# alibaba/PhotonLibOS

Measured on AMD Instinct MI355X. Metric: GiB/s CRC32C over device-resident buffers; % of HBM-read roofline, higher is better.
Workload: dtype u8; 1 GPU; C2: 65536 x 64 KiB random buffers, device-resident, per GPU; config=c2, buffers=65536, buffer_bytes=65536, parallelism=shard-per-gpu x1, lanes_per_buffer=auto

## Files before the change

### include/photon_crc/tuning.h

```cpp
#ifndef PHOTON_CRC_TUNING_H
#define PHOTON_CRC_TUNING_H

#include <stdint.h>

#ifdef __cplusplus
extern "C" {
#endif

int photon_crc_set_lanes_per_buffer(int g);

int photon_crc_set_batch_grid(int workgroups);

int photon_crc_set_generic_rows(int rows_per_step);

int photon_crc_set_msg_mode(int mode);

int photon_crc_set_msg_rows(int rows_per_step);

int photon_crc_set_mid_kernel(int on);

int photon_crc_set_long_shape(int lanes, int rounds);

int photon_crc64_set_full_rows(int mode, int rows_per_step);

int photon_crc_set_routed_wait(int spin_us, int sleep_ahead);

int photon_crc_set_small_service(int idle_us);
int photon_crc_set_small_service_life(int life_us);
int photon_crc_set_service_doorbell(int bar);
int photon_crc_small_service_doorbell(int kind);
int photon_crc_small_service_stats(uint64_t* served, uint64_t* starts, uint64_t* missed);
uint64_t photon_crc_small_service_deferred(void);

int photon_crc_lanes_for(uint64_t nbytes);

void photon_crc_test_fail_next(int n);

int photon_crc_test_tables(int which, uint32_t* out, int n);

int photon_crc_test_long_plan(uint64_t addr, uint64_t n, int cus, int lanes, int rounds, int crc64, uint64_t* out,
                              int nout);

int photon_crc_test_fold_parts(int crc64, const void* crc, const uint64_t* len, uint64_t count, uint64_t seed,
                               uint32_t nthreads, uint64_t* result, uint64_t* total);

int photon_crc_util_fold_on_host(int crc64, const void* d_crc, const uint64_t* h_len, const uint64_t* h_obj_start,
                                 uint64_t nobj, uint64_t nparts, uint64_t seed, void* h_out, void* stream);

int photon_crc_util_fill_splitmix(void* d_base, uint64_t stride, uint64_t nbytes, uint64_t count,
                                  uint64_t seed_base, void* stream);

int photon_crc_util_read_stream(const void* d_base, uint64_t nbytes, uint32_t* d_sink, uint64_t sink_words,
                                void* stream);

#ifdef __cplusplus
}
#endif

#endif
```

### photonlibos_amd/_native.py

```python
import ctypes
import os

_HERE = os.path.dirname(os.path.abspath(__file__))
LIB_PATH = os.environ.get("PHOTON_CRC_LIB") or os.path.join(_HERE, "lib", "libphoton_checksum.so")

_lib = None


class NativeLibraryMissing(ImportError):
    pass


class PhotonRange(ctypes.Structure):
    _fields_ = [("min", ctypes.c_int), ("max", ctypes.c_int)]


def lib():
    global _lib
    if _lib is None:
        if not os.path.exists(LIB_PATH):
            raise NativeLibraryMissing(
                f"{LIB_PATH} not found: build it with `python -c 'import __graft_entry__ as g; g.build()'` "
                "(or `make -C photonlibos_amd/csrc`)")
        _lib = ctypes.CDLL(LIB_PATH, mode=ctypes.RTLD_GLOBAL)
        _declare(_lib)
    return _lib


def _declare(L):
    u8p, u32, u64, sz, vp = ctypes.c_char_p, ctypes.c_uint32, ctypes.c_uint64, ctypes.c_size_t, ctypes.c_void_p
    u32p = ctypes.POINTER(ctypes.c_uint32)

    def fn(name, res, *args):
        f = getattr(L, name)
        f.restype = res
        f.argtypes = list(args)

    fn("photon_crc_device_count", ctypes.c_int)
    fn("photon_crc_last_error", ctypes.c_char_p)
    fn("photon_crc_scratch_release", ctypes.c_int64)
    fn("photon_crc_set_lanes_per_buffer", ctypes.c_int, ctypes.c_int)
    fn("photon_crc_set_batch_grid", ctypes.c_int, ctypes.c_int)
    fn("photon_crc32c_batch_strided", ctypes.c_int, vp, u64, u64, u64, u32, vp, vp, vp)
    fn("photon_crc32c_batch_strided_sync", ctypes.c_int, vp, u64, u64, u64, u32, vp, vp, vp)
    fn("photon_crc32c_batch_iov", ctypes.c_int, vp, u64, u32, vp, vp, vp)
    fn("photon_crc32c_host_batch_strided", ctypes.c_int, vp, u64, u64, u64, u32, vp, vp)
    fn("photon_crc32c_host_batch_strided_multi", ctypes.c_int, vp, u64, u64, u64, u32, vp, vp, ctypes.c_int)
    fn("photon_crc32c_batch_strided_shards", ctypes.c_int, vp, ctypes.c_int)
    fn("photon_crc32c_batch_msg", ctypes.c_int, vp, vp, u64, u32, vp, vp, vp, vp)
    fn("photon_crc32c_combine_batch", ctypes.c_int, vp, vp, vp, u64, vp, vp)
    fn("photon_crc64ecma_batch_strided", ctypes.c_int, vp, u64, u64, u64, u64, vp, vp, vp)
    fn("photon_crc64ecma_batch_iov", ctypes.c_int, vp, u64, u64, vp, vp, vp)
    fn("photon_crc64ecma_host_batch_strided", ctypes.c_int, vp, u64, u64, u64, u64, vp, vp)
    fn("photon_crc64ecma_trim_batch", ctypes.c_int, vp, vp, vp, u64, vp, vp, vp)
    fn("photon_crc64ecma_combine_batch", ctypes.c_int, vp, vp, vp, u64, vp, vp)
    fn("photon_crc64ecma_batch_msg_n", ctypes.c_int, vp, vp, u64, u64, u64, vp, vp, vp, vp)
    fn("photon_crc64ecma_extend_device", ctypes.c_int, vp, u64, u64, vp, vp)
    fn("photon_crc_util_fill_splitmix", ctypes.c_int, vp, u64, u64, u64, u64, vp)
    fn("photon_crc_util_read_stream", ctypes.c_int, vp, u64, vp, u64, vp)
    fn("photon_crc_set_generic_rows", ctypes.c_int, ctypes.c_int)
    fn("photon_crc_set_long_shape", ctypes.c_int, ctypes.c_int, ctypes.c_int)
    fn("photon_crc_set_msg_mode", ctypes.c_int, ctypes.c_int)
    fn("photon_crc_set_routed_wait", ctypes.c_int, ctypes.c_int, ctypes.c_int)
    fn("photon_crc_set_small_service", ctypes.c_int, ctypes.c_int)
    fn("photon_crc_set_mid_kernel", ctypes.c_int, ctypes.c_int)
    fn("photon_crc_small_service_stats", ctypes.c_int, vp, vp, vp)
    fn("photon_crc_set_small_service_life", ctypes.c_int, ctypes.c_int)
    fn("photon_crc_set_service_doorbell", ctypes.c_int, ctypes.c_int)
    fn("photon_crc_small_service_doorbell", ctypes.c_int, ctypes.c_int)
    fn("photon_crc_small_service_deferred", u64)
    fn("photon_crc64_set_full_rows", ctypes.c_int, ctypes.c_int, ctypes.c_int)
    fn("photon_crc_host_register", ctypes.c_int, vp, u64)
    fn("photon_crc_stream_create", ctypes.c_int, ctypes.POINTER(vp))
    fn("photon_crc_stream_destroy", ctypes.c_int, vp)
    fn("photon_crc_stream_sync", ctypes.c_int, vp)
    fn("photon_crc_stream_on_complete", ctypes.c_int, vp, vp, vp)
    fn("photon_crc_device_alloc", ctypes.c_int, ctypes.POINTER(vp), u64)
    fn("photon_crc_device_free", ctypes.c_int, vp)
    fn("photon_crc_memcpy_async", ctypes.c_int, vp, vp, u64, vp)
    fn("photon_crc_host_unregister", ctypes.c_int, vp)
    fn("photon_crc32c_file_strided", ctypes.c_int, ctypes.c_int, u64, u64, u64, u64, u32, vp)
    fn("photon_crc_dispatch_fallbacks", u64)
    fn("photon_crc_lanes_for", ctypes.c_int, u64)
    fn("photon_crc_test_fail_next", None, ctypes.c_int)
    fn("photon_crc_test_long_plan", ctypes.c_int, u64, u64, ctypes.c_int, ctypes.c_int, ctypes.c_int, ctypes.c_int,
       vp, ctypes.c_int)
    fn("photon_crc32c_series_device", ctypes.c_int, vp, u32, u32, vp, vp)
    fn("photon_crc32c_combine_series_device", ctypes.c_int, vp, u32, u32, vp, vp)
    fn("photon_crc32c_trim_batch", ctypes.c_int, vp, vp, vp, u64, vp, vp, vp)
    fn("photon_crc32c_extend_device", ctypes.c_int, vp, u64, u32, vp, vp)
    fn("photon_crc32c_extend_spans", ctypes.c_int, vp, ctypes.c_int, u32, vp)
    fn("photon_crc64ecma_extend_spans", ctypes.c_int, vp, ctypes.c_int, u64, vp)
    fn("photon_crc_set_device_dispatch", ctypes.c_int, ctypes.c_int)
    fn("photon_crc32c_batch_msg_n", ctypes.c_int, vp, vp, u64, u64, u32, vp, vp, vp, vp)
    fn("photon_crc32c_copy_batch_strided", ctypes.c_int, vp, u64, vp, u64, u64, u64, u32, vp, vp, vp)
    fn("photon_crc32c_copy_batch_iov", ctypes.c_int, vp, vp, u64, u32, vp, vp, vp)
    fn("photon_crc32c_gather_msg_n", ctypes.c_int, vp, vp, u64, u64, vp, u32, vp, vp, vp, vp)
    fn("photon_crc64ecma_copy_batch_strided", ctypes.c_int, vp, u64, vp, u64, u64, u64, u64, vp, vp, vp)
    fn("photon_crc64ecma_copy_batch_iov", ctypes.c_int, vp, vp, u64, u64, vp, vp, vp)
    fn("photon_crc64ecma_gather_msg_n", ctypes.c_int, vp, vp, u64, u64, vp, u64, vp, vp, vp, vp)
    fn("photon_crc32c_copy_msg_iov_n", ctypes.c_int, vp, vp, u64, vp, vp, u64, u64, vp, u32, vp, vp, vp, vp)
    fn("photon_crc64ecma_copy_msg_iov_n", ctypes.c_int, vp, vp, u64, vp, vp, u64, u64, vp, u64, vp, vp, vp, vp)
    fn("photon_crc32c_copy_msg_iov_seg_n", ctypes.c_int, vp, vp, u64, vp, vp, u64, u64, vp, u32, vp, ctypes.c_int, vp,
       vp, vp, vp)
    fn("photon_crc64ecma_copy_msg_iov_seg_n", ctypes.c_int, vp, vp, u64, vp, vp, u64, u64, vp, u64, vp, ctypes.c_int,
       vp, vp, vp, vp)
    fn("photon_crc32c_copy_extend_device", ctypes.c_int, vp, vp, u64, u32, vp, vp)
    fn("photon_crc64ecma_copy_extend_device", ctypes.c_int, vp, vp, u64, u64, vp, vp)
    fn("photon_crc64ecma_series_device", ctypes.c_int, vp, u32, u32, vp, vp)
    fn("photon_crc64ecma_combine_series_device", ctypes.c_int, vp, u32, u32, vp, vp)
    fn("photon_crc32c_fold_parts_n", ctypes.c_int, vp, vp, vp, u64, u64, u32, vp, vp, vp, vp)
    fn("photon_crc64ecma_fold_parts_n", ctypes.c_int, vp, vp, vp, u64, u64, u64, vp, vp, vp, vp)
    fn("photon_crc_test_fold_parts", ctypes.c_int, ctypes.c_int, vp, vp, u64, u64, u32, vp, vp)
    fn("photon_crc_util_fold_on_host", ctypes.c_int, ctypes.c_int, vp, vp, vp, u64, u64, u64, vp, vp)
    fn("photon_crc_pinned_allocate", ctypes.c_int, vp, PhotonRange, ctypes.POINTER(vp))
    fn("photon_crc_pinned_deallocate", ctypes.c_int, vp, vp)
    fn("photon_crc_pinned_stats", ctypes.c_int, ctypes.POINTER(u64), ctypes.POINTER(u64))
    fn("photon_crc_pinned_release", ctypes.c_int64)
    fn("photon_crc_msg_batch_create", vp, u32, u32, u32)
    fn("photon_crc_msg_batch_destroy", None, vp)
    fn("photon_crc_msg_batch_add", ctypes.c_int64, vp, vp, u32, vp, u64, u32)
    fn("photon_crc_msg_batch_submit", ctypes.c_int, vp, vp, vp, vp)
    fn("photon_crc_msg_batch_wait", ctypes.c_int64, vp)
    fn("photon_crc_msg_batch_result", ctypes.c_int, vp, u64, ctypes.POINTER(u32))
    fn("photon_crc_msg_batch_count", u64, vp)
    fn("photon_crc_msg_batch_reset", ctypes.c_int, vp)

    cpp = {
        "crc32c_sw": ("_Z9crc32c_swPKhmj", u32, u8p, sz, u32),
        "crc32c_hw": ("_Z9crc32c_hwPKhmj", u32, u8p, sz, u32),
        "crc32c_hw_simple": ("_Z16crc32c_hw_simplePKhmj", u32, u8p, sz, u32),
        "crc32c_hw_portable": ("_Z18crc32c_hw_portablePKhmj", u32, u8p, sz, u32),
        "crc32c_series_sw": ("_Z16crc32c_series_swPKhjjPj", None, u8p, u32, u32, u32p),
        "crc32c_series_hw": ("_Z16crc32c_series_hwPKhjjPj", None, u8p, u32, u32, u32p),
        "crc32c_combine_sw": ("_Z17crc32c_combine_swjjj", u32, u32, u32, u32),
        "crc32c_combine_hw": ("_Z17crc32c_combine_hwjjj", u32, u32, u32, u32),
        "crc32c_combine_series_sw": ("_Z24crc32c_combine_series_swPjjj", u32, u32p, u32, u32),
        "crc32c_combine_series_hw": ("_Z24crc32c_combine_series_hwPjjj", u32, u32p, u32, u32),
        "crc32c_trim_sw": ("_Z14crc32c_trim_sw16CRC32C_ComponentS_S_", u32, u64, u64, u64),
        "crc32c_trim_hw": ("_Z14crc32c_trim_hw16CRC32C_ComponentS_S_", u32, u64, u64, u64),
        "crc64ecma_sw": ("_Z12crc64ecma_swPKhmm", u64, u8p, sz, u64),
        "crc64ecma_hw": ("_Z12crc64ecma_hwPKhmm", u64, u8p, sz, u64),
        "crc64ecma_series_sw": ("_Z19crc64ecma_series_swPKhjjPm", None, u8p, u32, u32, ctypes.POINTER(u64)),
        "crc64ecma_series_hw": ("_Z19crc64ecma_series_hwPKhjjPm", None, u8p, u32, u32, ctypes.POINTER(u64)),
        "crc64ecma_combine_sw": ("_Z20crc64ecma_combine_swmmj", u64, u64, u64, u32),
        "crc64ecma_combine_hw": ("_Z20crc64ecma_combine_hwmmj", u64, u64, u64, u32),
        "crc64ecma_combine_series_sw": ("_Z27crc64ecma_combine_series_swPmjj", u64, ctypes.POINTER(u64), u32, u32),
        "crc64ecma_combine_series_hw": ("_Z27crc64ecma_combine_series_hwPmjj", u64, ctypes.POINTER(u64), u32, u32),
        "crc64ecma_trim_sw": ("_Z17crc64ecma_trim_sw19CRC64ECMA_ComponentS_S_", u64, u64, u64, u64, u64, u64, u64),
        "crc64ecma_trim_hw": ("_Z17crc64ecma_trim_hw19CRC64ECMA_ComponentS_S_", u64, u64, u64, u64, u64, u64, u64),
    }
    L.cpp = {}
    for py, (mangled, res, *args) in cpp.items():
        f = getattr(L, mangled)
# ... 9 lines not shown
```

### photonlibos_amd/checksum.py

```python
import ctypes

from ._native import lib

__all__ = [
    "CrcError",
    "crc32c", "crc32c_extend", "crc32c_sw", "crc32c_hw", "crc32c_hw_simple", "crc32c_hw_portable",
    "crc32c_series", "crc32c_series_sw", "crc32c_series_hw",
    "crc32c_combine", "crc32c_combine_sw", "crc32c_combine_hw",
    "crc32c_combine_series", "crc32c_combine_series_sw", "crc32c_combine_series_hw",
    "crc32c_trim", "crc32c_trim_sw", "crc32c_trim_hw", "is_crc32c_hw_available",
    "device_count", "set_lanes_per_buffer", "host_batch_strided", "host_batch_strided_multi", "batch_strided_shards",
    "Shard", "batch_strided", "batch_strided_sync", "batch_iov", "batch_msg",
    "copy_batch_strided", "copy_batch_iov", "gather_msg_n",
    "crc64ecma", "crc64ecma_extend", "crc64ecma_sw", "crc64ecma_hw", "crc64ecma_combine", "crc64ecma_series",
    "crc64ecma_combine_series", "crc64ecma_trim",
    "copy_batch64_strided", "copy_batch64_iov", "gather64_msg_n",
    "copy_msg_iov_n", "copy_msg64_iov_n",
    "copy_msg_iov_seg_n", "copy_msg64_iov_seg_n", "SEG_OF_SRC", "SEG_OF_DST",
    "copy_extend_device", "copy_extend64_device",
    "series64_device", "combine_series64_device", "fold_parts_device", "fold_parts64_device",
    "crc64ecma_series_at", "crc64ecma_combine_series_at",
    "batch64_strided", "batch64_iov", "combine64_batch", "trim64_batch", "batch64_msg_n", "host_batch64_strided", "extend64_device", "extend_spans", "extend64_spans", "Span", "combine_batch", "fill_splitmix", "read_stream", "IOVEC_DTYPE",
]

# ... 490 lines not shown


_SERIES64_PTR_FN = _SERIES_PTR_FN
_CSER64_PTR_FN = ctypes.CFUNCTYPE(ctypes.c_uint64, ctypes.c_void_p, ctypes.c_uint32, ctypes.c_uint32)


def crc64ecma_series_at(addr, part_size, n_parts, out_addr):
    _auto("crc64ecma_series_auto", _SERIES64_PTR_FN)(addr, part_size, n_parts, out_addr)


def crc64ecma_combine_series_at(addr, part_size, n_parts):
    return _auto("crc64ecma_combine_series_auto", _CSER64_PTR_FN)(addr, part_size, n_parts)


def host_register(addr, nbytes):
    _check(lib().photon_crc_host_register(addr, nbytes))


def host_unregister(addr):
    _check(lib().photon_crc_host_unregister(addr))


def file_strided(fd, offset, stride, nbytes, count, seed=0):
    out = (ctypes.c_uint32 * max(count, 1))()
    _check(lib().photon_crc32c_file_strided(fd, offset, stride, nbytes, count, seed & 0xFFFFFFFF, out))
    return list(out)[:count]


def set_generic_rows(u):
    _check(lib().photon_crc_set_generic_rows(u))


def set_msg_mode(mode):
    _check(lib().photon_crc_set_msg_mode(mode))


def set_long_shape(lanes=0, rounds=0):
    _check(lib().photon_crc_set_long_shape(lanes, rounds))


def set_routed_wait(spin_us=40, sleep_ahead=True):
    _check(lib().photon_crc_set_routed_wait(spin_us, 1 if sleep_ahead else 0))


def set_mid_kernel(on=True):
    _check(lib().photon_crc_set_mid_kernel(1 if on else 0))


def set_small_service(idle_us):
    _check(lib().photon_crc_set_small_service(int(idle_us)))


def set_small_service_life(life_us):
    _check(lib().photon_crc_set_small_service_life(int(life_us)))


def set_service_doorbell(bar):
    _check(lib().photon_crc_set_service_doorbell(1 if bar else 0))


def small_service_doorbell(kind=0):
    r = lib().photon_crc_small_service_doorbell(int(kind))
    if r == -2:
        return None
    _check(r if r < 0 else 0)
    return "bar" if r == 1 else "pinned"


def small_service_deferred():
    return int(lib().photon_crc_small_service_deferred())


def small_service_stats():
    import ctypes
    v = [ctypes.c_uint64(0) for _ in range(3)]
    _check(lib().photon_crc_small_service_stats(*[ctypes.byref(x) for x in v]))
    return tuple(x.value for x in v)


def set_full_rows64(mode, rows_per_step=2):
    _check(lib().photon_crc64_set_full_rows(mode, rows_per_step))


def set_msg_rows(u):
    _check(lib().photon_crc_set_msg_rows(u))


def read_stream(base, nbytes, sink, sink_words, stream=None):
    _check(lib().photon_crc_util_read_stream(_ptr(base), nbytes, _ptr(sink), sink_words, _stream(stream)))


def fill_splitmix(base, stride, nbytes, count, seed_base, stream=None):
    _check(lib().photon_crc_util_fill_splitmix(_ptr(base), stride, nbytes, count, seed_base, _stream(stream)))


def scratch_release():
    return int(lib().photon_crc_scratch_release())
```

### photonlibos_amd/csrc/crc32c_device.hip

```cpp
#include <hip/hip_runtime.h>

#include <errno.h>
#include <fcntl.h>
#include <stdint.h>
#include <stdio.h>
#include <string.h>

#include <sys/prctl.h>
#include <unistd.h>

#include <atomic>
#include <chrono>
#include <memory>
#include <map>
#include <tuple>
#include <mutex>
#include <string>
#include <thread>
#include <type_traits>
#include <vector>

#include <photon/common/checksum/crc32c.h>
#include <photon/common/checksum/crc64ecma.h>

#include "../../include/photon_crc/crc32c_gpu.h"
#include "../../include/photon_crc/tuning.h"
#include "crc32c_kernels.h"
#include "crc64_kernels.h"
#include "long_plan.h"
#include "multi_device.h"
#include "gf2.h"
#include "internal.h"

namespace pcrc {
int host_engine_table(int which, uint32_t* out, int n);

namespace {

thread_local std::string g_err;

std::atomic<int> g_lanes_override{0};
std::atomic<int> g_grid_cap{0};
std::atomic<int> g_generic_u{-1};
std::atomic<int> g_msg_u{2};
std::atomic<int> g_msg_mode{0};
std::atomic<uint32_t> g_full64{2u << 4 | 3u};
std::atomic<uint32_t> g_routed_wait{40u | 1u << 16};
constexpr int kSvcIdleDefault = 200;
int svc_idle_from_env() {
    const char* e = getenv("PHOTON_CRC_SMALL_SERVICE");
    if (!e || !*e) return kSvcIdleDefault;
    const long v = strtol(e, nullptr, 10);
    return v < 0 ? 0 : v > 1000000 ? 1000000 : (int)v;
}
std::atomic<int> g_svc_idle_us{svc_idle_from_env()};
std::atomic<int> g_svc_life_us{2000};
int svc_bell_from_env() {
    const char* e = getenv("PHOTON_CRC_SVC_DOORBELL");
    return e && (!strcmp(e, "host") || !strcmp(e, "pinned") || !strcmp(e, "0")) ? 0 : 1;
}
std::atomic<int> g_svc_bell{svc_bell_from_env()};
std::atomic<uint64_t> g_svc_served{0}, g_svc_starts{0}, g_svc_missed{0}, g_svc_deferred{0};
std::atomic<int> g_svc_made{0};
void service_end_all();
void svc_yield();
void heavy_mark(hipStream_t st);

struct HeavyLaunch {
    hipStream_t st;
    explicit HeavyLaunch(hipStream_t s) : st(s) { svc_yield(); }
    ~HeavyLaunch() { heavy_mark(st); }
};
int service_doorbell_of(int dev, int kind);

int fail(int code, const std::string& what) {
    g_err = what;
    return code;
}

int hip_fail(hipError_t e, const char* what, const char* rest = "") {
    return fail(-EIO, std::string(what) + rest + ": " + hipGetErrorString(e));
}

struct HipRT {
    int get(int* dev) {
        const hipError_t e = hipGetDevice(dev);
        return e == hipSuccess ? 0 : hip_fail(e, "hipGetDevice");
    }
    int set(int dev) {
        const hipError_t e = hipSetDevice(dev);
        return e == hipSuccess ? 0 : hip_fail(e, "hipSetDevice");
    }
};

struct DeviceInfo {
    bool probed = false;
    bool ok = false;
    int cus = 0;
};

std::mutex g_mu;
std::vector<DeviceInfo> g_dev;
thread_local int g_fail_next = 0;

void table_images_init();

int current_device(int* cus) {
    if (g_fail_next > 0) {
        --g_fail_next;
        return fail(-EIO, "injected failure (photon_crc_test_fail_next)");
    }
    int dev = 0;
    hipError_t e = hipGetDevice(&dev);
    if (e != hipSuccess) return hip_fail(e, "hipGetDevice");
    std::lock_guard<std::mutex> lk(g_mu);
    if ((int)g_dev.size() <= dev) g_dev.resize(dev + 1);
    DeviceInfo& di = g_dev[dev];
    if (!di.probed) {
        hipDeviceProp_t prop;
        e = hipGetDeviceProperties(&prop, dev);
        if (e != hipSuccess) return hip_fail(e, "hipGetDeviceProperties");
        di.ok = strncmp(prop.gcnArchName, "gfx950", 6) == 0;
        di.cus = prop.multiProcessorCount;
        di.probed = true;
        if (!di.ok) g_err = std::string("device is ") + prop.gcnArchName + ", need gfx950";
        if (di.ok) table_images_init();
    }
    if (!di.ok) return fail(-ENODEV, "photon_crc: no gfx950 device (got other arch)");
    *cus = di.cus;
// ... 108 lines not shown
    c.kshift = xpow(8ull * 16ull * (uint64_t)b * (uint64_t)g);
    mul_basis(c.kshift, c.sbasis);
    for (int k = 0; k < 6; ++k) mul_basis(xpow((128ull * (uint64_t)b) << k), c.basis[k]);
    for (int d = 0; d < 8; ++d) mul_basis(xpow(32ull + 128ull * (uint64_t)d), c.fbasis[d]);
    return c;
}

const LaneConsts& lane_consts(int g, int b = 1) {
    static LaneConsts tab[7][3];
    static std::once_flag once;
    std::call_once(once, [] {
        for (int lg = 2; lg <= 6; ++lg)
            for (int lb = 0; lb <= 2; ++lb) tab[lg][lb] = make_lane_consts(1 << lg, 1 << lb);
    });
    const int lg = g == 64 ? 6 : g == 32 ? 5 : g == 16 ? 4 : g == 8 ? 3 : 2;
    const int lb = b == 4 ? 2 : b == 2 ? 1 : 0;
    return tab[lg][lb];
}

LaneConsts64 make_lane_consts64(int g) {
    LaneConsts64 c;
    c.kshift = xpow64(8ull * 16ull * (uint64_t)g);
    for (int i = 0; i < 64; ++i) c.sbasis[i] = mulmod64(1ull << i, c.kshift);
    return c;
}

const LaneConsts64& lane_consts64(int g) {
    static LaneConsts64 tab[7];
    static std::once_flag once;
    std::call_once(once, [] {
        for (int lg = 2; lg <= 6; ++lg) tab[lg] = make_lane_consts64(1 << lg);
    });
    return tab[g == 64 ? 6 : g == 32 ? 5 : g == 16 ? 4 : g == 8 ? 3 : 2];
}

template <typename W>
typename W::Pow squarings(typename W::T v) {
    typename W::Pow t;
    for (int i = 0; i < 64; ++i) {
        t.x8pow2[i] = v;
        v = W::mul(v, v);
    }
    return t;
}

template <typename W, bool INV>
const typename W::Pow& x8_table() {
    static typename W::Pow t;
    static std::once_flag once;
    std::call_once(once, [] { t = squarings<W>(INV ? W::xpow_inv(8) : W::xpow(8)); });
    return t;
}

template <typename W>
const typename W::Pow& pow_table() {
    return x8_table<W, false>();
}

template <typename W>
const typename W::Pow& rshift_table() {
    return x8_table<W, true>();
}

template <typename W>
typename W::Pow part_pow_table(uint64_t part) {
    return squarings<W>(W::xpow(8ull * part));
}

int choose_lanes(uint64_t typical_len) {
    if (const int g = g_lanes_override.load(std::memory_order_relaxed)) return g;
    if (typical_len >= (512u << 10)) return 64;
    if (typical_len >= (32u << 10)) return 32;
    if (typical_len >= 2048) return 8;
    return 4;
}

int batch_lanes(uint64_t typical_len) {
    if (const int g = g_lanes_override.load(std::memory_order_relaxed)) return g;
    if (typical_len >= 4096 && typical_len < 8192) return 16;
    return choose_lanes(typical_len);
}

constexpr int default_rows(int g) { return g == 16 ? 2 : 4; }

int batch_rows(int g) {
    const int u = g_generic_u.load(std::memory_order_relaxed);
    return u >= 0 ? u : default_rows(g);
}

std::vector<uint32_t> small_image_host();
std::vector<uint64_t> small64_image_host();

struct Crc32c : Gf32 {
    static constexpr const char* kKernel = "crc32c";
    static constexpr const char* kExtend = "crc32c_extend";
    static constexpr const char* kSeries = "crc32c_series";
    static constexpr const char* kCombineSeries = "crc32c_combine_series";
    static constexpr const char* kCombineSeriesLaunch = "combine_series kernel launch";
    static constexpr bool kCrc64 = false;
    static constexpr int kService = 0;
    typedef LaneConsts Lanes;
    typedef PowTable Pow;
    typedef BatchArgs Batch;
    typedef CopyBatchArgs CopyBatch;
    typedef CopyIovArgs CopyIov;
    typedef SmallArgs Small;
    typedef LongArgs Long;
    typedef CopyLongArgs CopyLong;
    static T xpow(uint64_t n) { return pcrc::xpow(n); }
    static T xpow_inv(uint64_t n) { return pcrc::xpow_inv(n); }
    static const Lanes& lanes(int g) { return lane_consts(g); }
    static constexpr bool kShiftInit = PCRC_SHIFT_INIT;
    static T shift_init(T seed0, uint64_t nbytes) { return mul(seed0, xpow(8ull * nbytes)); }
    static int copy_lanes(uint64_t typical_len) { return batch_lanes(typical_len); }
    static constexpr uint32_t kSeriesMinPart = 8;
    static constexpr uint32_t kSeedBytes = 4;
    static void put_seed(Small* a, T seed) { a->seed = seed; }
    static T seed_word(const Small& a) { return a.seed; }
    static constexpr uint32_t kImageBytes = kSmImage;
    static constexpr const char* kImageName = "small-buffer table image";
    static std::vector<T> image_host() { return small_image_host(); }
    static constexpr uint32_t kMidBlocks = pcrc::kMidBlocks, kMidRows = pcrc::kMidRows;
    template <uint32_t V, int R>
    static auto small_kernel() { return &crc32c_small_kernel<V, R>; }
    template <int G>
    static auto long_kernel() { return &crc32c_long_kernel<G, 4>; }
    template <int G>
    static auto copy_long_kernel() { return &crc32c_copy_long_kernel<G, 4>; }
    static void long_args(Long* a, const LongPlan& lp, const LongPowers& pw, const void* data, T seed, T* out) {
        pcrc::long_args(a, lp, pw, data, seed, out);
    }
    static constexpr auto* kCombineKernel = &crc32c_combine_kernel;
    static constexpr auto* kTrimKernel = &crc32c_trim_kernel;
    static constexpr auto* kFoldPartsKernel = &crc32c_fold_parts_kernel;
    static constexpr auto* kCombineSeriesKernel = &crc32c_combine_series_kernel;
    static bool combine_series_of_empty(const T* d_crc, uint32_t part_size, uint32_t n_parts, T* d_result,
                                        hipStream_t st) {
        if (part_size) return false;
        hipLaunchKernelGGL(crc32c_first_nonzero_kernel, dim3(1), dim3(1024), 0, st, d_crc, (uint64_t)n_parts,
                           d_result);
        return true;
    }
    static constexpr uint32_t kWords = 1;
    static T routed_result(const uint32_t* x, bool ) { return x[0]; }
    static void routed_diag(char* buf, size_t n, const volatile uint64_t* w, uint32_t tag) {
        snprintf(buf, n, "; word %016llx, tag %08x", (unsigned long long)w[0], tag);
    }
    static inline T (*host_crc)(const uint8_t*, size_t, T) = nullptr;
    static inline void (*host_series)(const uint8_t*, uint32_t, uint32_t, T*) = nullptr;
    static inline T (*host_cseries)(T*, uint32_t, uint32_t) = nullptr;
};

struct Crc64 : Gf64 {
    static constexpr const char* kKernel = "crc64";
    static constexpr const char* kExtend = "crc64ecma_extend";
    static constexpr const char* kSeries = "crc64ecma_series";
    static constexpr const char* kCombineSeries = "crc64ecma_combine_series";
    static constexpr const char* kCombineSeriesLaunch = "crc64_combine_series_kernel launch";
    static constexpr bool kCrc64 = true;
    static constexpr int kService = 1;
    typedef LaneConsts64 Lanes;
    typedef PowTable64 Pow;
    typedef Batch64Args Batch;
    typedef CopyBatch64Args CopyBatch;
    typedef CopyIov64Args CopyIov;
    typedef Small64Args Small;
    typedef Long64Args Long;
    typedef CopyLong64Args CopyLong;
    static T xpow(uint64_t n) { return xpow64(n); }
    static T xpow_inv(uint64_t n) { return xpow64_inv(n); }
    static const Lanes& lanes(int g) { return lane_consts64(g); }
    static constexpr bool kShiftInit = PCRC64_SHIFT_INIT;
    static T shift_init(T seed0, uint64_t nbytes) { return mul(~seed0, xpow(8ull * nbytes)); }
    static int copy_lanes(uint64_t typical_len) { return choose_lanes(typical_len); }
    static constexpr uint32_t kSeriesMinPart = 1;
    static constexpr uint32_t kSeedBytes = 8;
    static void put_seed(Small* a, T seed) { a->init = ~seed; }
    static T seed_word(const Small& a) { return a.init; }
    static constexpr uint32_t kImageBytes = kSm64Image;
    static constexpr const char* kImageName = "CRC-64 small-buffer table image";
    static std::vector<T> image_host() { return small64_image_host(); }
    static constexpr uint32_t kMidBlocks = kMid64Blocks, kMidRows = kMid64Rows;
    template <uint32_t V, int R>
    static auto small_kernel() { return &crc64_small_kernel<V, R>; }
    template <int G>
    static auto long_kernel() { return &crc64_long_kernel<G>; }
    template <int G>
    static auto copy_long_kernel() { return &crc64_copy_long_kernel<G>; }
    static void long_args(Long* a, const LongPlan& lp, const LongPowers& pw, const void* data, T seed, T* out) {
        long_args64(a, lp, pw, data, seed, out);
    }
    static constexpr auto* kCombineKernel = &crc64_combine_kernel;
    static constexpr auto* kTrimKernel = &crc64_trim_kernel;
    static constexpr auto* kFoldPartsKernel = &crc64_fold_parts_kernel;
    static constexpr auto* kCombineSeriesKernel = &crc64_combine_series_kernel;
    static bool combine_series_of_empty(const T*, uint32_t, uint32_t, T*, hipStream_t) { return false; }
    static constexpr uint32_t kWords = 2;
    static T routed_result(const uint32_t* x, bool raw) {
        const T v = ((T)x[1] << 32) | x[0];
        return raw ? ~v : v;
    }
    static void routed_diag(char* buf, size_t n, const volatile uint64_t* w, uint32_t tag) {
        snprintf(buf, n, "; words %016llx %016llx, tag %08x", (unsigned long long)w[0], (unsigned long long)w[1],
                 tag);
    }
    static inline T (*host_crc)(const uint8_t*, size_t, T) = nullptr;
    static inline void (*host_series)(const uint8_t*, uint32_t, uint32_t, T*) = nullptr;
    static inline T (*host_cseries)(T*, uint32_t, uint32_t) = nullptr;
};

uint64_t batch_grid(uint64_t units, int g, int cus, bool capped) {
    const uint64_t gpw = 64 / (uint64_t)g;
    const uint64_t waves = (units + gpw - 1) / gpw;
    uint64_t grid = (waves + kWaves - 1) / kWaves;
    if (grid > (uint64_t)cus) grid = cus;
    if (capped)
        if (const int cap = g_grid_cap.load(std::memory_order_relaxed))
            grid = grid > (uint64_t)cap ? (uint64_t)cap : grid;
    return grid;
}

template <int N>
using Int = std::integral_constant<int, N>;

template <typename F>
void with_lanes(int g, F f) {
    switch (g) {
        case 64: f(Int<64>{}); break;
        case 32: f(Int<32>{}); break;
        case 16: f(Int<16>{}); break;
        case 8: f(Int<8>{}); break;
        default: f(Int<4>{}); break;
    }
}

template <typename W, typename L>
int launch_lanes(uint64_t units, int g, bool capped, hipStream_t stream, const char* what, L launch) {
    if (units == 0) return 0;
    int cus = 0;
    int dev = current_device(&cus);
    if (dev < 0) return dev;
    const dim3 grid(batch_grid(units, g, cus, capped));
    const typename W::Lanes& kc = W::lanes(g);
    HeavyLaunch heavy(stream);
    with_lanes(g, [&](auto G) { launch(G, grid, kc); });
    const hipError_t e = hipGetLastError();
    return e == hipSuccess ? 0 : hip_fail(e, what);
}

int launch_batch(const BatchArgs& a, uint64_t typical_len, hipStream_t stream, int lanes = 0) {
    const int g = lanes ? lanes : batch_lanes(typical_len);
    const int rows_per_step = batch_rows(g);
    return launch_lanes<Crc32c>(a.count, g, true, stream, "crc32c_batch_kernel launch",
                                [&](auto G, dim3 grid, const LaneConsts& kc) {
        auto rows = [&](auto U) {
            hipLaunchKernelGGL((crc32c_batch_kernel<decltype(G)::value, decltype(U)::value>), grid, dim3(kBlock), 0,
                               stream, a, kc, pow_table<Crc32c>());
        };
        if (rows_per_step == 2)
            rows(Int<2>{});
        else if (rows_per_step == 8)
            rows(Int<8>{});
        else
            rows(Int<4>{});
    });
}

int launch_copy(const CopyBatchArgs& a, uint64_t units, int g, hipStream_t stream, int msg = 0) {
    return launch_lanes<Crc32c>(units, g, true, stream, "crc32c_batch_kernel<copy> launch",
                                [&](auto G, dim3 grid, const LaneConsts& kc) {
        constexpr int GG = decltype(G)::value, U = default_rows(GG);
        if (msg == 2)
            hipLaunchKernelGGL((crc32c_batch_kernel<GG, U, 2, true>), grid, dim3(kBlock), 0, stream, a, kc,
                               pow_table<Crc32c>());
        else if (msg == 1)
            hipLaunchKernelGGL((crc32c_batch_kernel<GG, U, 1, true>), grid, dim3(kBlock), 0, stream, a, kc,
                               pow_table<Crc32c>());
        else
            hipLaunchKernelGGL((crc32c_batch_kernel<GG, U, 0, true>), grid, dim3(kBlock), 0, stream, a, kc,
                               pow_table<Crc32c>());
    });
}

int launch_copy_iov(const CopyIovArgs& a, int g, hipStream_t stream) {
    return launch_lanes<Crc32c>(a.nmsg, g, true, stream, "crc32c_copy_iov_kernel launch",
                                [&](auto G, dim3 grid, const LaneConsts& kc) {
        constexpr int GG = decltype(G)::value;
        hipLaunchKernelGGL((crc32c_copy_iov_kernel<GG, default_rows(GG)>), grid, dim3(kBlock), 0, stream, a, kc);
    });
}

int launch_copy_iov_seg(const CopyIovSegArgs& a, bool dst_side, int g, hipStream_t stream) {
    return launch_lanes<Crc32c>(a.nmsg, g, true, stream, "crc32c_copy_iov_seg_kernel launch",
                                [&](auto G, dim3 grid, const LaneConsts& kc) {
        constexpr int GG = decltype(G)::value, U = default_rows(GG);
        if (dst_side)
            hipLaunchKernelGGL((crc32c_copy_iov_seg_kernel<GG, U, true>), grid, dim3(kBlock), 0, stream, a, kc,
                               pow_table<Crc32c>());
        else
            hipLaunchKernelGGL((crc32c_copy_iov_seg_kernel<GG, U, false>), grid, dim3(kBlock), 0, stream, a, kc,
                               pow_table<Crc32c>());
    });
}

int launch_batch(const Batch64Args& a, uint64_t typical_len, hipStream_t stream) {
    int g = choose_lanes(typical_len);
    const uint32_t full = g_full64.load(std::memory_order_relaxed);
    const int fu = (full & 15u) == 3u ? (typical_len >= 8192 ? 4 : 2) : (int)(full >> 4);
    auto full_rows = [&](int gg) {
        const int fx = (full & 15u) == 3u ? (gg <= 16 ? 2 : 0) : (int)(full & 15u);
        return fx && !a.iov && a.shift_init && a.nbytes % (2ull * 16ull * (uint64_t)gg * (uint64_t)fu) == 0 ? fx : 0;
    };
    if (!g_lanes_override.load(std::memory_order_relaxed) && typical_len >= 4096 && typical_len <= 8192)
        g = full_rows(8) ? 8 : 16;
    const int fx = full_rows(g);
    return launch_lanes<Crc64>(a.count, g, false, stream, fx ? "crc64_full_kernel launch" : "crc64_batch_kernel launch",
                               [&](auto G, dim3 grid, const LaneConsts64& kc) {
        constexpr int GG = decltype(G)::value;
        auto full = [&](auto U) {
            constexpr int UU = decltype(U)::value;
            if (fx == 2)
                hipLaunchKernelGGL((crc64_full_kernel<GG, UU, true>), grid, dim3(kBlock), 0, stream, a, kc);
            else
                hipLaunchKernelGGL((crc64_full_kernel<GG, UU, false>), grid, dim3(kBlock), 0, stream, a, kc);
        };
        if (!fx)
            hipLaunchKernelGGL(crc64_batch_kernel<GG>, grid, dim3(kBlock), 0, stream, a, kc);
        else if (fu == 4)
            full(Int<4>{});
        else
            full(Int<2>{});
    });
}

template <typename L>
int launch_copying64(uint64_t units, int g, hipStream_t stream, const char* what, L launch) {
#if PCRC64_ABL != 0 || PCRC64_ROLL != 1 || PCRC64_U != 2
    (void)launch;
    return units == 0 ? 0 : fail(-ENOTSUP, "the copying CRC-64 kernels are not part of this A/B build");
// ... 723 lines not shown
}

int photon_crc_test_tables(int which, uint32_t* out, int n) {
    if (!out) return fail(-EINVAL, "null output");
    if (which <= 3 || which == 8) {
        const int rc = host_engine_table(which, out, n);
        return rc < 0 ? fail(-EINVAL, "bad table id or short output") : rc;
    }
    if (n < 32) return fail(-EINVAL, "short output");
    if (which == 4 || which == 5) {
        const PowTable& t = which == 4 ? pow_table<Crc32c>() : rshift_table<Crc32c>();
        for (int i = 0; i < 32; ++i) out[i] = t.x8pow2[i];
        return 32;
    }
    if (which == 6) {
        for (int k = 0; k < 5; ++k) out[k] = lane_consts(4 << k).kshift;
        return 5;
    }
    if (which == 7) {
        const LaneConsts& c = lane_consts(64);
        for (int k = 0; k < 6; ++k) out[k] = c.basis[k][31];
        return 6;
    }
    if (which == 9) {
        const LaneConsts& c = lane_consts(8);
        for (int d = 0; d < 8; ++d) out[d] = c.fbasis[d][31];
        return 8;
    }
    return fail(-EINVAL, "bad table id");
}

int photon_crc_test_long_plan(uint64_t addr, uint64_t n, int cus, int lanes, int rounds, int crc64, uint64_t* out,
                              int nout) {
    if (!out || cus < 1 || (lanes != 0 && lanes != 32 && lanes != 64) || rounds < 0 || rounds > 64)
        return fail(-EINVAL, "bad plan arguments");
    const LongPlan lp = long_plan_for(reinterpret_cast<const void*>(addr), n, cus,
                                      (uint32_t)lanes | (uint32_t)rounds << 8, 0, crc64 != 0);
    const LongPowers& pw = long_powers(lp, crc64 != 0);
    std::vector<uint64_t> w = {lp.head, lp.chunk, lp.nchunks, lp.last, lp.rounds, lp.grid, lp.stride, lp.lead,
                               (uint64_t)lp.lanes};
    if (crc64) {
        w.insert(w.end(), pw.xsb64, pw.xsb64 + 64);
        w.push_back(pw.x64);
        w.insert(w.end(), pw.zt64, pw.zt64 + 16);
        w.insert(w.end(), pw.ft64, pw.ft64 + lp.grid);
    } else {
        w.insert(w.end(), pw.xsb32, pw.xsb32 + 32);
        w.insert(w.end(), pw.xb32, pw.xb32 + 32);
        w.insert(w.end(), pw.zt32, pw.zt32 + 16);
        w.insert(w.end(), pw.ft32, pw.ft32 + lp.grid);
    }
    if ((int)w.size() > nout) return fail(-EINVAL, "short output");
    memcpy(out, w.data(), w.size() * 8);
    return (int)w.size();
}

int photon_crc_set_generic_rows(int rows_per_step) {
    if (rows_per_step != -1 && rows_per_step != 2 && rows_per_step != 4 && rows_per_step != 8)
        return fail(-EINVAL, "rows per step must be -1 (auto), 2, 4 or 8");
    g_generic_u.store(rows_per_step, std::memory_order_relaxed);
    return 0;
}

int photon_crc_set_msg_mode(int mode) {
    if (mode < 0 || mode > 2) return fail(-EINVAL, "message mode must be 0 (auto), 1 (fused) or 2 (two kernels)");
    g_msg_mode.store(mode, std::memory_order_relaxed);
    return 0;
}

int photon_crc_set_long_shape(int lanes, int rounds) {
    if ((lanes != 0 && lanes != 32 && lanes != 64) || rounds < 0 || rounds > 64)
        return fail(-EINVAL, "long-buffer lanes must be 0, 32 or 64 and rounds 0..64");
    g_long_shape.store((uint32_t)lanes | (uint32_t)rounds << 8, std::memory_order_relaxed);
    return 0;
}

int photon_crc64_set_full_rows(int mode, int rows_per_step) {
    if (mode < 0 || mode > 3 || (rows_per_step != 2 && rows_per_step != 4))
        return fail(-EINVAL, "full-row mode must be 0..3 and rows per step 2 or 4");
    g_full64.store((uint32_t)rows_per_step << 4 | (uint32_t)mode, std::memory_order_relaxed);
    return 0;
}

int photon_crc_set_routed_wait(int spin_us, int sleep_ahead) {
    if (spin_us < 0 || spin_us > 65535) return fail(-EINVAL, "spin window must be 0..65535 us");
    g_routed_wait.store((uint32_t)spin_us | (sleep_ahead ? 1u << 16 : 0u), std::memory_order_relaxed);
    return 0;
}

int photon_crc_set_small_service(int idle_us) {
    if (idle_us < 0 || idle_us > 1000000) return fail(-EINVAL, "service idle time must be 0..1000000 us");
    g_svc_idle_us.store(idle_us, std::memory_order_relaxed);
    if (idle_us == 0) service_end_all();
    return 0;
}

int photon_crc_set_small_service_life(int life_us) {
    if (life_us < 100 || life_us > 1000000) return fail(-EINVAL, "service life must be 100..1000000 us");
    g_svc_life_us.store(life_us, std::memory_order_relaxed);
    return 0;
}

int photon_crc_set_service_doorbell(int bar) {
    if (bar != 0 && bar != 1) return fail(-EINVAL, "doorbell must be 0 (pinned host) or 1 (device BAR)");
    service_end_all();
    g_svc_bell.store(bar, std::memory_order_relaxed);
    return 0;
}

int photon_crc_small_service_doorbell(int kind) {
    if (kind != 0 && kind != 1) return fail(-EINVAL, "kind must be 0 (CRC-32C) or 1 (CRC-64)");
    int dev = 0;
    if (hipGetDevice(&dev) != hipSuccess) return fail(-ENODEV, "no device");
    return service_doorbell_of(dev, kind);
}

uint64_t photon_crc_small_service_deferred(void) { return g_svc_deferred.load(std::memory_order_relaxed); }

int photon_crc_small_service_stats(uint64_t* served, uint64_t* starts, uint64_t* missed) {
    if (served) *served = g_svc_served.load(std::memory_order_relaxed);
    if (starts) *starts = g_svc_starts.load(std::memory_order_relaxed);
    if (missed) *missed = g_svc_missed.load(std::memory_order_relaxed);
    return 0;
}

int photon_crc_set_msg_rows(int rows_per_step) {
    if (rows_per_step != 2 && rows_per_step != 4) return fail(-EINVAL, "message rows per step must be 2 or 4");
    g_msg_u.store(rows_per_step, std::memory_order_relaxed);
    return 0;
}

int photon_crc32c_batch_strided(const void* d_base, uint64_t stride, uint64_t nbytes, uint64_t count,
                                uint32_t seed0, const uint32_t* d_seeds, uint32_t* d_out, void* stream) {
    return batch_strided<Crc32c>(d_base, stride, nbytes, count, seed0, d_seeds, d_out, stream);
}

int photon_crc32c_batch_strided_sync(const void* d_base, uint64_t stride, uint64_t nbytes, uint64_t count,
                                     uint32_t seed0, const uint32_t* d_seeds, uint32_t* d_out, void* stream) {
    int rc = photon_crc32c_batch_strided(d_base, stride, nbytes, count, seed0, d_seeds, d_out, stream);
    if (rc) return rc;
    hipError_t e = hipStreamSynchronize(static_cast<hipStream_t>(stream));
    if (e != hipSuccess) return hip_fail(e, "hipStreamSynchronize");
    return 0;
}

}

namespace pcrc {
namespace {

template <typename T>
int host_batch_impl(const void* h_base, uint64_t stride, uint64_t nbytes, uint64_t count, T seed0, const T* h_seeds,
                    T* h_out,
                    int (*device_batch)(const void*, uint64_t, uint64_t, uint64_t, T, const T*, T*, void*)) {
    if (!count) return 0;
    if (!h_out || (!h_base && nbytes) || stride < nbytes) return fail(-EINVAL, "bad arguments");
    if (!nbytes) {
        for (uint64_t i = 0; i < count; ++i) h_out[i] = h_seeds ? h_seeds[i] : seed0;
        return 0;
    }
    const uint64_t pitch = (nbytes + 255) & ~uint64_t(255);
    if (pitch > kStageBytes) return fail(-EINVAL, "buffer larger than a staging chunk (256 MiB)");
    int cus = 0;
    int dev = current_device(&cus);
    if (dev < 0) return dev;
    if (dev >= kMaxDevices) return fail(-ENODEV, "device index beyond the pipeline table");
// ... 1342 lines not shown
```

### photonlibos_amd/csrc/crc32c_kernels.h

```cpp
#pragma once
#include <hip/hip_runtime.h>
#include <stdint.h>

#include <type_traits>

#include "../../include/photon_crc/crc32c_gpu.h"
#include "fold_parts.h"
#include "gf2.h"

#ifndef PCRC_LANE_SEL
#define PCRC_LANE_SEL 1
#endif
#ifndef PCRC_LONG_LEAD
#define PCRC_LONG_LEAD true
#endif
#ifndef PCRC_LONG_MERGE_HEAD
#define PCRC_LONG_MERGE_HEAD 1
#endif
#ifndef PCRC_BATCH_LEAD
#define PCRC_BATCH_LEAD false
#endif
#ifndef PCRC_BATCH_LEAD2
#define PCRC_BATCH_LEAD2 true
#endif
// ... 872 lines not shown
        if (bi < args.count) {
            if (args.iov) {
                *p = static_cast<const uint8_t*>(args.iov[bi].base);
                *n = args.iov[bi].len;
            } else {
                *p = args.base + bi * args.stride;
                *n = args.nbytes;
            }
            if (args.seeds) *seed = args.seeds[bi];
        }
    };
    auto copy_item = [&](uint64_t wv, const uint8_t* p, uint64_t n) {
        CopyTo ct;
        if constexpr (COPY) {
            const uint64_t bi = wv * GPW + grp;
            if (bi < args.count) {
                uint8_t* dst = args.dst ? static_cast<uint8_t*>(args.dst[bi]) : args.dst_base + bi * args.dst_stride;
                ct = copy_begin<G>(p, dst, n, gl);
            }
        }
        return ct;
    };
    if constexpr (kOverlap) {
        constexpr uint32_t kVec = lds_bytes_for<G>() / 16, kPer = (kVec + kBlock - 1) / kBlock;
        const uint32_t* img = g_table_image[table_slot<G>()];
        const uint32_t tid = threadIdx.x;
        u32x4 tv[kPer];
        if (img && !(PCRC_ABL & 4)) {
#pragma unroll
            for (uint32_t i = 0; i < kPer; ++i) {
                const uint32_t j = i * kBlock + tid;
                tv[i] = j < kVec ? *((const g_u32x4*)img + j) : u32x4{0, 0, 0, 0};
            }
        }
        uint64_t wv = (uint64_t)blockIdx.x * kWaves + wave;
        const uint8_t* p;
        uint64_t n;
        uint32_t seed;
        item(wv, &p, &n, &seed);
        BufGeo g = buf_geo<G>(p, n, gl);
        BufPre<U, kLead> pre;
        if (wv * GPW < args.count) buf_preload<G, U, kLead>(g, gl, pre);
        if (PCRC_ABL & 4) {
            lds_barrier();
        } else if (img) {
#pragma unroll
            for (uint32_t i = 0; i < kPer; ++i) {
                const uint32_t j = i * kBlock + tid;
                if (j < kVec) *reinterpret_cast<u32x4*>(lds + 4 * j) = tv[i];
            }
            lds_barrier();
        } else {
            build_tables<G>(lds, kc);
        }
        for (bool first = true; wv * GPW < args.count; wv += nwaves, first = false) {
            if (!first) {
                item(wv, &p, &n, &seed);
                g = buf_geo<G>(p, n, gl);
                buf_preload<G, U, kLead>(g, gl, pre);
            }
            const uint32_t s = args.shift_init ? 0u : seed;
            const CopyTo ct = copy_item(wv, p, n);
            const uint32_t pc = buf_body<G, U, kLead, COPY>(lds, g, pre, s, gl, la, !args.shift_init, ct);
            const uint32_t crc = buf_finish<G, COPY>(lds, g, pc, p, n, s, gl, la, ct);
            const uint64_t bi = wv * GPW + grp;
            if (bi < args.count && gl == 0) args.out[bi] = crc ^ args.init_shift;
        }
        return;
    }
    for (uint64_t wv = (uint64_t)blockIdx.x * kWaves + wave; wv * GPW < args.count; wv += nwaves) {
        const uint64_t bi = wv * GPW + grp;
        const bool active = bi < args.count;
        const uint8_t* p;
        uint64_t n;
        uint32_t seed;
        item(wv, &p, &n, &seed);
        const CopyTo ct = copy_item(wv, p, n);
        const uint32_t crc = buffer_crc<G, U, kLead, COPY>(lds, p, n, args.shift_init ? 0u : seed, gl, la,
                                                           !args.shift_init, ct);
        if (active && gl == 0) args.out[bi] = crc ^ args.init_shift;
    }
}

struct CopyIovArgs {
    const photon_crc_iovec* src;
    const uint64_t* src_start;
    const photon_crc_iovec* dst;
    const uint64_t* dst_start;
    uint64_t nmsg;
    const uint64_t* size;
    const uint32_t* seeds;
    uint32_t* out;
    uint64_t* copied;
    uint32_t seed0;
};

template <bool PF>
struct IovCursor {
    const photon_crc_iovec* v;
    uint64_t i, end;
    const uint8_t* p;
    uint64_t rem;
    photon_crc_iovec nx[PF ? 1 : 0];
    __device__ __forceinline__ void take(const photon_crc_iovec& c) {
        p = static_cast<const uint8_t*>(c.base);
        rem = c.len;
        if constexpr (PF) nx[0] = v[i + 1 < end ? i + 1 : i];
    }
    __device__ __forceinline__ void begin(const photon_crc_iovec* iov, uint64_t s0, uint64_t s1) {
        v = iov;
        i = s0;
        end = s1;
        p = nullptr;
        rem = 0;
        if constexpr (PF) nx[0] = {nullptr, 0};
        if (s0 < s1) take(iov[s0]);
    }
    __device__ __forceinline__ bool more() const { return i < end; }
    __device__ __forceinline__ void next() {
        if (++i < end) {
            if constexpr (PF) take(nx[0]);
            else take(v[i]);
        }
    }
};

template <int G, int U>
__global__ __launch_bounds__(kBlock) void crc32c_copy_iov_kernel(CopyIovArgs args, LaneConsts kc) {
    __shared__ __attribute__((aligned(16))) uint32_t lds[lds_bytes_for<G>() / 4];
    constexpr bool kMsgLead = PCRC_MSG_LEAD != 0;
    load_tables<G>(lds, kc);

    constexpr int GPW = 64 / G;
    const uint32_t lane = threadIdx.x & 63u;
    const uint32_t wave = wave_id();
    const uint32_t gl = lane & (G - 1);
    const uint32_t grp = lane / G;
    const LaneAddr la = lane_addr(lane);

    const uint64_t nwaves = (uint64_t)gridDim.x * kWaves;
    for (uint64_t wv = (uint64_t)blockIdx.x * kWaves + wave; wv * GPW < args.nmsg; wv += nwaves) {
        const uint64_t m = wv * GPW + grp;
        const bool active = m < args.nmsg;
        uint32_t acc = args.seed0;
        uint64_t left = 0;
        IovCursor<true> s, d;
        s.begin(args.src, 0, 0);
        d.begin(args.dst, 0, 0);
        if (active) {
            left = args.size ? args.size[m] : ~0ull;
            if (args.seeds) acc = args.seeds[m];
            s.begin(args.src, args.src_start[m], args.src_start[m + 1]);
            d.begin(args.dst, args.dst_start[m], args.dst_start[m + 1]);
        }
        while (left && s.more() && d.more()) {
            uint64_t n = s.rem < d.rem ? s.rem : d.rem;
            n = n < left ? n : left;
            const CopyTo ct = copy_begin<G>(s.p, const_cast<uint8_t*>(d.p), n, gl);
            acc = buffer_crc<G, U, kMsgLead, true>(lds, s.p, n, acc, gl, la, true, ct);
            s.p += n;
            d.p += n;
            s.rem -= n;
            d.rem -= n;
            left -= n;
            if (!left) break;
            if (!s.rem) s.next();
// ... 1034 lines not shown
```

Baseline: 6401 GiB/s.

## Add specialized full-row CRC32C kernel for uniform aligned strided batches

```diff
diff --git a/include/photon_crc/tuning.h b/include/photon_crc/tuning.h
--- a/include/photon_crc/tuning.h
+++ b/include/photon_crc/tuning.h
@@ -22,6 +22,11 @@
 int photon_crc_set_long_shape(int lanes, int rounds);
 
 int photon_crc64_set_full_rows(int mode, int rows_per_step);
+
+int photon_crc32c_set_full_rows(int mode);
+
+int photon_crc32c_full_rows_for(uint64_t base_addr, uint64_t stride, uint64_t nbytes, int has_seeds, int* lanes,
+                                int* rows);
 
 int photon_crc_set_routed_wait(int spin_us, int sleep_ahead);
 
diff --git a/photonlibos_amd/_native.py b/photonlibos_amd/_native.py
--- a/photonlibos_amd/_native.py
+++ b/photonlibos_amd/_native.py
@@ -70,6 +70,9 @@
     fn("photon_crc_small_service_doorbell", ctypes.c_int, ctypes.c_int)
     fn("photon_crc_small_service_deferred", u64)
     fn("photon_crc64_set_full_rows", ctypes.c_int, ctypes.c_int, ctypes.c_int)
+    fn("photon_crc32c_set_full_rows", ctypes.c_int, ctypes.c_int)
+    fn("photon_crc32c_full_rows_for", ctypes.c_int, u64, u64, u64, ctypes.c_int, ctypes.POINTER(ctypes.c_int),
+       ctypes.POINTER(ctypes.c_int))
     fn("photon_crc_host_register", ctypes.c_int, vp, u64)
     fn("photon_crc_stream_create", ctypes.c_int, ctypes.POINTER(vp))
     fn("photon_crc_stream_destroy", ctypes.c_int, vp)
diff --git a/photonlibos_amd/checksum.py b/photonlibos_amd/checksum.py
--- a/photonlibos_amd/checksum.py
+++ b/photonlibos_amd/checksum.py
@@ -596,6 +596,17 @@
     _check(lib().photon_crc64_set_full_rows(mode, rows_per_step))
 
 
+def set_full_rows32(mode):
+    _check(lib().photon_crc32c_set_full_rows(mode))
+
+
+def full_rows_for(base, stride, nbytes, has_seeds=False):
+    g, u = ctypes.c_int(0), ctypes.c_int(0)
+    mode = lib().photon_crc32c_full_rows_for(base, stride, nbytes, 1 if has_seeds else 0, ctypes.byref(g),
+                                             ctypes.byref(u))
+    return int(mode), g.value, u.value
+
+
 def set_msg_rows(u):
     _check(lib().photon_crc_set_msg_rows(u))
 
diff --git a/photonlibos_amd/csrc/crc32c_device.hip b/photonlibos_amd/csrc/crc32c_device.hip
--- a/photonlibos_amd/csrc/crc32c_device.hip
+++ b/photonlibos_amd/csrc/crc32c_device.hip
@@ -45,6 +45,11 @@
 std::atomic<int> g_msg_u{2};
 std::atomic<int> g_msg_mode{0};
 std::atomic<uint32_t> g_full64{2u << 4 | 3u};
+int full32_from_env() {
+    const char* e = getenv("PHOTON_CRC32C_FULL_ROWS");
+    return e && e[0] >= '0' && e[0] <= '3' && !e[1] ? e[0] - '0' : 3;
+}
+std::atomic<int> g_full32{full32_from_env()};
 std::atomic<uint32_t> g_routed_wait{40u | 1u << 16};
 constexpr int kSvcIdleDefault = 200;
 int svc_idle_from_env() {
@@ -319,11 +324,6 @@
 }
 
 constexpr int default_rows(int g) { return g == 16 ? 2 : 4; }
-
-int batch_rows(int g) {
-    const int u = g_generic_u.load(std::memory_order_relaxed);
-    return u >= 0 ? u : default_rows(g);
-}
 
 std::vector<uint32_t> small_image_host();
 std::vector<uint64_t> small64_image_host();
@@ -485,13 +485,57 @@
     return e == hipSuccess ? 0 : hip_fail(e, what);
 }
 
+struct FullRows32 {
+    int mode, rows;
+};
+
+FullRows32 full_rows32_auto(int g) {
+    if (g == 64) return {2, 2};
+    return {0, 0};
+}
+
+FullRows32 full_rows32(bool uniform, uint64_t nbytes, int g) {
+    const int mode = g_full32.load(std::memory_order_relaxed);
+    const int ku = g_generic_u.load(std::memory_order_relaxed);
+    const FullRows32 generic{0, ku >= 0 ? ku : default_rows(g)};
+    if (!mode || !uniform || g < 8) return generic;
+    FullRows32 f{mode, generic.rows};
+    if (mode == 3) {
+        if (ku >= 0) return generic;
+        f = full_rows32_auto(g);
+        if (!f.mode) return generic;
+    }
+    if (f.rows != 2 && f.rows != 4) return generic;
+    const uint64_t step = 16ull * (uint64_t)g * (uint64_t)f.rows;
+    if (nbytes == 0 || nbytes % (2 * step) || nbytes / step > 0xffffffffull) return generic;
+    return f;
+}
+
 int launch_batch(const BatchArgs& a, uint64_t typical_len, hipStream_t stream, int lanes = 0) {
     const int g = lanes ? lanes : batch_lanes(typical_len);
-    const int rows_per_step = batch_rows(g);
-    return launch_lanes<Crc32c>(a.count, g, true, stream, "crc32c_batch_kernel launch",
+    const FullRows32 fr = full_rows32(!a.iov && !a.msg_start && a.shift_init, a.nbytes, g);
+    const int rows_per_step = fr.rows, fx = fr.mode;
+    return launch_lanes<Crc32c>(a.count, g, true, stream, fx ? "crc32c_full_kernel launch" : "crc32c_batch_kernel launch",
                                 [&](auto G, dim3 grid, const LaneConsts& kc) {
+        constexpr int GG = decltype(G)::value;
+        auto full = [&](auto U) {
+            constexpr int UU = decltype(U)::value;
+            if constexpr (GG >= 8) {
+                if (fx == 2)
+                    hipLaunchKernelGGL((crc32c_full_kernel<GG, UU, true>), grid, dim3(kBlock), 0, stream, a, kc);
+                else
+                    hipLaunchKernelGGL((crc32c_full_kernel<GG, UU, false>), grid, dim3(kBlock), 0, stream, a, kc);
+            }
+        };
+        if (fx) {
+            if (rows_per_step == 2)
+                full(Int<2>{});
+            else
+                full(Int<4>{});
+            return;
+        }
         auto rows = [&](auto U) {
-            hipLaunchKernelGGL((crc32c_batch_kernel<decltype(G)::value, decltype(U)::value>), grid, dim3(kBlock), 0,
+            hipLaunchKernelGGL((crc32c_batch_kernel<GG, decltype(U)::value>), grid, dim3(kBlock), 0,
                                stream, a, kc, pow_table<Crc32c>());
         };
         if (rows_per_step == 2)
@@ -1381,6 +1425,22 @@
     return 0;
 }
 
+int photon_crc32c_set_full_rows(int mode) {
+    if (mode < 0 || mode > 3) return fail(-EINVAL, "full-row mode must be 0..3");
+    g_full32.store(mode, std::memory_order_relaxed);
+    return 0;
+}
+
+int photon_crc32c_full_rows_for(uint64_t base_addr, uint64_t stride, uint64_t nbytes, int has_seeds, int* lanes,
+                                int* rows) {
+    const bool uniform = Crc32c::kShiftInit && !has_seeds && !(base_addr & 15) && !(stride & 15) && nbytes >= 64;
+    const int g = batch_lanes(nbytes);
+    const FullRows32 fr = full_rows32(uniform, nbytes, g);
+    if (lanes) *lanes = g;
+    if (rows) *rows = fr.rows;
+    return fr.mode;
+}
+
 int photon_crc_set_routed_wait(int spin_us, int sleep_ahead) {
     if (spin_us < 0 || spin_us > 65535) return fail(-EINVAL, "spin window must be 0..65535 us");
     g_routed_wait.store((uint32_t)spin_us | (sleep_ahead ? 1u << 16 : 0u), std::memory_order_relaxed);
diff --git a/photonlibos_amd/csrc/crc32c_kernels.h b/photonlibos_amd/csrc/crc32c_kernels.h
--- a/photonlibos_amd/csrc/crc32c_kernels.h
+++ b/photonlibos_amd/csrc/crc32c_kernels.h
@@ -978,6 +978,86 @@
     }
 }
 
+template <int U, bool FIRST>
+__device__ __forceinline__ uint32_t full_column_fold(const uint32_t* lds, uint32_t q, const uint32_t (&c)[U],
+                                                     const LaneAddr& a) {
+    if constexpr (FIRST) q = c[0];
+#pragma unroll
+    for (int u = FIRST ? 1 : 0; u < U; ++u) q = sstep(lds, q, a, c[u]);
+    return q;
+}
+
+template <int G, int U, bool FIRST>
+__device__ __forceinline__ uint32_t full_roll_step(const uint32_t* lds, uint32_t q, uint4 (&cur)[U],
+                                                   const uint8_t* next, const LaneAddr& a) {
+    uint32_t c[U];
+#pragma unroll
+    for (int u = 0; u < U; ++u) {
+        c[u] = lag16(lds, cur[u], a);
+        cur[u] = load16(next + u * (16 * G));
+    }
+    return full_column_fold<U, FIRST>(lds, q, c, a);
+}
+
+template <int U>
+__device__ __forceinline__ uint32_t full_last_step(const uint32_t* lds, uint32_t q, const uint4 (&cur)[U],
+                                                   const LaneAddr& a) {
+    uint32_t c[U];
+#pragma unroll
+    for (int u = 0; u < U; ++u) c[u] = lag16(lds, cur[u], a);
+    return full_column_fold<U, false>(lds, q, c, a);
+}
+
+template <int G, int U>
+__device__ __forceinline__ void load_step(uint4 (&w)[U], const uint8_t* p) {
+#pragma unroll
+    for (int u = 0; u < U; ++u) w[u] = load16(p + u * (16 * G));
+}
+
+template <int G, int U, bool XB>
+__global__ __launch_bounds__(kBlock) void crc32c_full_kernel(BatchArgs args, LaneConsts kc) {
+    __shared__ __attribute__((aligned(16))) uint32_t lds[lds_bytes_for<G>() / 4];
+    load_tables<G>(lds, kc);
+    constexpr int GPW = 64 / G;
+    constexpr uint32_t kStep = 16u * G * U;
+    const uint32_t lane = threadIdx.x & 63u;
+    const uint32_t gl = lane & (G - 1);
+    const uint32_t grp = lane / G;
+    const LaneAddr la = lane_addr(lane);
+    const uint64_t nwaves = (uint64_t)gridDim.x * kWaves;
+    const uint32_t steps = __builtin_amdgcn_readfirstlane((uint32_t)(args.nbytes / kStep));
+    uint64_t wv = (uint64_t)blockIdx.x * kWaves + wave_id();
+    if (wv * GPW >= args.count) return;
+    auto lane_ptr = [&](uint64_t w) {
+        const uint64_t bi = w * GPW + grp;
+        return args.base + (bi < args.count ? bi : args.count - 1) * args.stride + 16u * gl;
+    };
+    uint4 cur[U];
+    const uint8_t* p = lane_ptr(wv);
+    load_step<G, U>(cur, p);
+    for (;;) {
+        const uint64_t next = wv + nwaves;
+        const bool more = next * GPW < args.count;
+        const uint8_t* pn = more ? lane_ptr(next) : p;
+        uint32_t pc = full_roll_step<G, U, true>(lds, 0u, cur, p + kStep, la);
+        if constexpr (XB) {
+            for (uint32_t s = 1; s < steps; ++s)
+                pc = full_roll_step<G, U, false>(lds, pc, cur, s + 1 < steps ? p + (uint64_t)(s + 1) * kStep : pn, la);
+        } else {
+            for (uint32_t s = 1; s + 1 < steps; ++s)
+                pc = full_roll_step<G, U, false>(lds, pc, cur, p + (uint64_t)(s + 1) * kStep, la);
+            pc = full_last_step<U>(lds, pc, cur, la);
+        }
+        const uint32_t crc = finish_group<G>(lds, pc, G - 1 - gl, la) ^ args.init_shift;
+        const uint64_t bi = wv * GPW + grp;
+        if (gl == 0 && bi < args.count) args.out[bi] = crc;
+        if (!more) break;
+        if constexpr (!XB) load_step<G, U>(cur, pn);
+        wv = next;
+        p = pn;
+    }
+}
+
 struct CopyIovArgs {
     const photon_crc_iovec* src;
     const uint64_t* src_start;
```

Result: no change. 6401 GiB/s, median of 2 (-0.0%).
